# nianticlabs/simplerecon

Hardware: AMD Instinct MI355X
Metric: depth frames/sec (640x480, 7 src views, 64 planes) (higher is better)
Workload: dtype f32

## Files before the change

simplerecon_amd/csrc/sr_common.h:

```cpp
#pragma once
#include <hip/hip_runtime.h>
#include <stdint.h>

#include "simplerecon_hip.h"

#define SR_GEOM_STRIDE 20

#define SR_WAVE 64

int sr_opt(int id);

int sr_device_cus();

static inline int sr_hip_rc(hipError_t e) { return e == hipSuccess ? SR_OK : SR_ERR_HIP_BASE + (int)e; }

static inline size_t sr_align_up(size_t v, size_t a) { return (v + a - 1) / a * a; }

struct SrPlanes {
  const float* ptr;
  int64_t sb, sd, sy, sx;
};

struct SrVolumeOut {
  float* cv;
  int64_t sb, sd, sp;
  float* lowest;
  uint8_t* mask;
};

struct SrSample {
  float zp;
  float pix_x, pix_y;
  float w_nw, w_ne, w_sw, w_se;
  int o_nw, o_ne, o_sw, o_se;
};

typedef float sr_f2v __attribute__((ext_vector_type(2)));

__device__ __forceinline__ void sr_bilinear_taps(float ix, float iy, int h, int w, float& fx0, float& fy0, float& w_nw,
                                                 float& w_ne, float& w_sw, float& w_se) {
#pragma clang fp contract(off)
  const sr_f2v ixy = {ix, iy};
  fx0 = floorf(ix);
  fy0 = floorf(iy);
  const sr_f2v f0 = {fx0, fy0};
  const sr_f2v f1 = f0 + 1.0f;
  const float fx1 = f1.x, fy1 = f1.y;
  const float wm = (float)(w - 1), hm = (float)(h - 1);
  const bool vx0 = (fx0 >= 0.0f) & (fx0 <= wm), vx1 = (fx1 >= 0.0f) & (fx1 <= wm);
  const bool vy0 = (fy0 >= 0.0f) & (fy0 <= hm), vy1 = (fy1 >= 0.0f) & (fy1 <= hm);
  const sr_f2v a1 = f1 - ixy, a0 = ixy - f0;
  const sr_f2v wtop = sr_f2v{a1.x, a0.x} * a1.y;
  const sr_f2v wbot = sr_f2v{a1.x, a0.x} * a0.y;
  w_nw = (vx0 & vy0) ? wtop.x : 0.0f;
  w_ne = (vx1 & vy0) ? wtop.y : 0.0f;
  w_sw = (vx0 & vy1) ? wbot.x : 0.0f;
  w_se = (vx1 & vy1) ? wbot.y : 0.0f;
}

struct SrSampleXY {
  float zp, pix_x, pix_y;
  float ix, iy;
  float fx0, fy0;
  float w_nw, w_ne, w_sw, w_se;
};

__device__ __forceinline__ void sr_project_sample_xy(const float* __restrict__ g ,
                                                     float X0, float X1, float X2, int h, int w,
                                                     float inv_w, float inv_h, SrSampleXY& s) {
#pragma clang fp contract(off)
  const float eps = 1e-8f;
  const sr_f2v q01 = sr_f2v{g[0], g[4]} * X0 + sr_f2v{g[1], g[5]} * X1 + sr_f2v{g[2], g[6]} * X2 + sr_f2v{g[3], g[7]};
  const float q2 = g[8] * X0 + g[9] * X1 + g[10] * X2 + g[11];
  s.zp = q2 + eps;
  const float sc = (fabsf(q2) > eps) ? 1.0f / s.zp : 1.0f;
  const sr_f2v pix = q01 * sc;
  s.pix_x = pix.x;
  s.pix_y = pix.y;
  const sr_f2v uv = 2.0f * pix * sr_f2v{inv_w, inv_h} - 1.0f;
  const sr_f2v size = {(float)w, (float)h};
  const sr_f2v ixy = ((uv + 1.0f) * size - 1.0f) / 2.0f;
  s.ix = ixy.x;
  s.iy = ixy.y;
  sr_bilinear_taps(s.ix, s.iy, h, w, s.fx0, s.fy0, s.w_nw, s.w_ne, s.w_sw, s.w_se);
}

__device__ __forceinline__ void sr_project_sample(const float* __restrict__ g ,
                                                  float X0, float X1, float X2, int h, int w,
                                                  float inv_w, float inv_h, SrSample& s) {
  SrSampleXY c;
  sr_project_sample_xy(g, X0, X1, X2, h, w, inv_w, inv_h, c);
  s.zp = c.zp; s.pix_x = c.pix_x; s.pix_y = c.pix_y;
  s.w_nw = c.w_nw; s.w_ne = c.w_ne; s.w_sw = c.w_sw; s.w_se = c.w_se;
  const float wm = (float)(w - 1), hm = (float)(h - 1);
  const float fx1 = c.fx0 + 1.0f, fy1 = c.fy0 + 1.0f;
  const int x0 = (int)fminf(fmaxf(c.fx0, 0.0f), wm), x1 = (int)fminf(fmaxf(fx1, 0.0f), wm);
  const int y0 = (int)fminf(fmaxf(c.fy0, 0.0f), hm), y1 = (int)fminf(fmaxf(fy1, 0.0f), hm);
  s.o_nw = y0 * w + x0;
  s.o_ne = y0 * w + x1;
  s.o_sw = y1 * w + x0;
  s.o_se = y1 * w + x1;
}

__device__ __forceinline__ bool sr_in_bounds(const SrSample& s, int h, int w) {
  return (s.pix_x > 2.0f) & (s.pix_x < (float)(w - 2)) & (s.pix_y > 2.0f) & (s.pix_y < (float)(h - 2));
}

#ifdef __HIPCC__
__device__ __forceinline__ float sr_vmax(float a, float b) {
  float r;
  asm("v_max_f32 %0, %1, %2" : "=v"(r) : "v"(a), "v"(b));
  return r;
}
__device__ __forceinline__ float sr_vmin(float a, float b) {
  float r;
  asm("v_min_f32 %0, %1, %2" : "=v"(r) : "v"(a), "v"(b));
  return r;
}
__device__ __forceinline__ float sr_vmax_mfma(float a, float b) {
  float r;
  asm("v_max_f32 %0, %1, %2\n\ts_nop 1" : "=v"(r) : "v"(a), "v"(b));
  return r;
}
__device__ __forceinline__ float sr_activate(float v, float slope) {
  if (slope >= 0.0f) return fmaxf(v, 0.0f) + slope * fminf(v, 0.0f);
  if (slope < -1.5f) return v / (1.0f + __expf(-v));
  return v;
}
__device__ __forceinline__ float sr_uniform(float x) {
  return __builtin_bit_cast(float, __builtin_amdgcn_readfirstlane(__builtin_bit_cast(int, x)));
}
template <int N>
__device__ __forceinline__ void sr_activate_group(float (&v)[N], float slope) {
  if (slope >= 0.0f) {
    if (slope <= 1.0f) {
#pragma unroll
      for (int i = 0; i < N; ++i) v[i] = sr_vmax(v[i], slope * v[i]);
    } else {
#pragma unroll
      for (int i = 0; i < N; ++i) v[i] = sr_vmax(v[i], 0.0f) + slope * sr_vmin(v[i], 0.0f);
    }
  } else if (slope < -1.5f) {
#pragma unroll
    for (int i = 0; i < N; ++i) v[i] = v[i] / (1.0f + __expf(-v[i]));
  }
}
#endif

struct SrDotParams {
  const float* cur;
  const float* src_nhwc;
  const float* invK;
  const float* geom;
  SrPlanes planes;
  SrVolumeOut out;
  int B, K, h, w, D;
  float inv_w, inv_h;
};

static inline float* sr_ws_geom(void* workspace) { return (float*)sr_align_up((size_t)workspace, 256); }
static inline float* sr_ws_src_nhwc(void* workspace, int B, int K) {
  return (float*)((char*)sr_ws_geom(workspace) + sr_align_up((size_t)B * K * SR_GEOM_STRIDE * sizeof(float), 256));
}

static inline size_t sr_ws_nhwc_bytes(int B, int K, int C, int h, int w) {
  return sr_align_up((size_t)B * K * h * w * C * sizeof(float), 256);
}
static inline unsigned long long* sr_ws_keys(void* workspace, int B, int K, int C, int h, int w) {
  return (unsigned long long*)((char*)sr_ws_src_nhwc(workspace, B, K) + sr_ws_nhwc_bytes(B, K, C, h, w));
}

int sr_launch_dot_volume_lds(const SrDotParams& p, unsigned long long* keys, hipStream_t stream);
int sr_launch_geom(const float* K_src, const float* T_src_cur, const float* T_cur_src, float* geom,
                   int n, hipStream_t stream);
int sr_launch_argmax_planes(const float* cv, int64_t sb, int64_t sd, int64_t sp, SrPlanes planes, int B, int h, int w,
                            int D, float* lowest, hipStream_t stream);
int sr_launch_splitk_reduce(const float* part, int ksplit, int64_t part_stride, const float* bias, const float* res,
                            int64_t res_sb, int res_sp, float* out, int64_t out_sb, int out_sp, int B, int HW, int Cout,
                            float slope, hipStream_t stream);
int sr_launch_unpack_nhwc(const float* src_nhwc, float* dst_nchw, int images, int C, int npix, hipStream_t stream);
int sr_launch_pack_nhwc(const float* src_nchw, float* dst_nhwc, int images, int C, int npix,
                        hipStream_t stream);
```

simplerecon_amd/csrc/sr_mlp_volume.hip:

```cpp
#include <stdlib.h>
#include <string.h>

#include "sr_common.h"

typedef float f32x16 __attribute__((ext_vector_type(16)));

#define SR_HID 128
#define SR_VIEW_SLOTS 24
#define SR_INV_FIXED 20
#define SR_PLANE_CHUNK 8

static inline int sr_mlp_steps_var(int K) { return (SR_VIEW_SLOTS / 2) * K; }
static inline int sr_mlp_steps_inv(int K) { return (SR_INV_FIXED + 3 * K + 1) / 2; }
static inline int sr_mlp_steps1(int K) { return sr_mlp_steps_var(K) + sr_mlp_steps_inv(K); }
#define SR_MLP_STEPS2 65

static inline size_t sr_mlp_packed_floats(int K) { return (size_t)(sr_mlp_steps1(K) + SR_MLP_STEPS2) * 256 + 128 + 4; }

__global__ void sr_mlp_pack_kernel(const float* __restrict__ W1, const float* __restrict__ b1,
                                   const float* __restrict__ W2, const float* __restrict__ b2,
                                   const float* __restrict__ W3, const float* __restrict__ b3,
                                   float* __restrict__ packed, int K, int C) {
  const int steps_var = (SR_VIEW_SLOTS / 2) * K;
  const int steps1 = steps_var + (SR_INV_FIXED + 3 * K + 1) / 2;
  const int Cin = C * (K + 1) + 10 * K + 4;
  const int o_cur = K * C, o_mask = o_cur + C, o_z = o_mask + K, o_d = o_z + K, o_dot = o_d + 1;
  const int o_ang = o_dot + K, o_cray = o_ang + K, o_sray = o_cray + 3, o_pd = o_sray + 3 * K;
  const int o_rm = o_pd + K, o_tm = o_rm + K;
  const int total = (steps1 + SR_MLP_STEPS2) * 256 + 128 + 1;
  for (int e = blockIdx.x * blockDim.x + threadIdx.x; e < total; e += gridDim.x * blockDim.x) {
    float v = 0.0f;
    if (e < steps1 * 256) {
      const int t = e >> 8, lane = (e >> 2) & 63, mt = e & 3;
      const int row = 32 * mt + (lane & 31);
      int col = -1;
      if (t < steps_var) {
        const int slot = 2 * t + (lane >> 5);
        const int k = slot / SR_VIEW_SLOTS, s = slot - k * SR_VIEW_SLOTS;
        if (s < 16) col = k * C + s;
        else if (s == 16) col = o_mask + k;
        else if (s == 17) col = o_z + k;
        else if (s == 18) col = o_dot + k;
        else if (s == 19) col = o_ang + k;
        else if (s < 23) col = o_sray + 3 * k + (s - 20);
        else col = (k == 0) ? o_d : -1;
      } else {
        const int u = 2 * (t - steps_var) + (lane >> 5);
        if (u < 16) col = o_cur + u;
        else if (u < 19) col = o_cray + (u - 16);
        else if (u == 19) col = -2;
        else if (u < SR_INV_FIXED + 3 * K) {
          const int k = (u - SR_INV_FIXED) / 3, i = (u - SR_INV_FIXED) - 3 * k;
          col = (i == 0 ? o_pd : (i == 1 ? o_rm : o_tm)) + k;
        }
      }
      v = (col >= 0) ? W1[(size_t)row * Cin + col] : (col == -2 ? b1[row] : 0.0f);
    } else if (e < (steps1 + SR_MLP_STEPS2) * 256) {
      const int e2 = e - steps1 * 256;
      const int t = e2 >> 8, lane = (e2 >> 2) & 63, mt = e2 & 3;
      const int row = 32 * mt + (lane & 31);
      if (t < 64) {
        const int m = t >> 4, r = t & 15;
        const int f = 32 * m + (r & 3) + 8 * (r >> 2) + 4 * (lane >> 5);
        v = W2[(size_t)row * SR_HID + f];
      } else {
        v = (lane < 32) ? b2[row] : 0.0f;
      }
    } else if (e < (steps1 + SR_MLP_STEPS2) * 256 + 128) {
      const int i = e - (steps1 + SR_MLP_STEPS2) * 256;
      const int half = i >> 6, mt = (i >> 4) & 3, r = i & 15;
      v = W3[32 * mt + (r & 3) + 8 * (r >> 2) + 4 * half];
    } else {
      v = b3[0];
    }
    packed[e] = v;
  }
}


struct SrMlpParams {
  const float* cur;
  const float* src_nhwc;
  const float* invK;
  const float* geom;
  const float* packed;
  SrPlanes planes;
  SrVolumeOut out;
  int B, K, h, w, D;
  int tiles;
  int chunk, chunks;
  int vec_store;
  float inv_w, inv_h, slope;
};

__device__ __forceinline__ void sr_swap_halves(float fa, float fb, float& bP, float& bQ) {
  auto r = __builtin_amdgcn_permlane32_swap(__float_as_uint(fa), __float_as_uint(fb), false, false);
  bP = __uint_as_float(r[0]);
  bQ = __uint_as_float(r[1]);
}

#define SR_MFMA(a, b, c) __builtin_amdgcn_mfma_f32_32x32x2f32((a), (b), (c), 0, 0, 0)

__device__ __forceinline__ void sr_l1_step(f32x16 (&acc)[2][4], const float4 wA, float fa, float fb) {
  float bP, bQ;
  sr_swap_halves(fa, fb, bP, bQ);
  acc[0][0] = SR_MFMA(wA.x, bP, acc[0][0]);
  acc[1][0] = SR_MFMA(wA.x, bQ, acc[1][0]);
  acc[0][1] = SR_MFMA(wA.y, bP, acc[0][1]);
  acc[1][1] = SR_MFMA(wA.y, bQ, acc[1][1]);
  acc[0][2] = SR_MFMA(wA.z, bP, acc[0][2]);
  acc[1][2] = SR_MFMA(wA.z, bQ, acc[1][2]);
  acc[0][3] = SR_MFMA(wA.w, bP, acc[0][3]);
  acc[1][3] = SR_MFMA(wA.w, bQ, acc[1][3]);
}

__device__ __forceinline__ void sr_l1_step_init(f32x16 (&acc)[2][4], const f32x16 (&hc)[2][4], const float4 wA,
                                                float fa, float fb) {
  float bP, bQ;
  sr_swap_halves(fa, fb, bP, bQ);
  acc[0][0] = SR_MFMA(wA.x, bP, hc[0][0]);
  acc[1][0] = SR_MFMA(wA.x, bQ, hc[1][0]);
  acc[0][1] = SR_MFMA(wA.y, bP, hc[0][1]);
  acc[1][1] = SR_MFMA(wA.y, bQ, hc[1][1]);
  acc[0][2] = SR_MFMA(wA.z, bP, hc[0][2]);
  acc[1][2] = SR_MFMA(wA.z, bQ, hc[1][2]);
  acc[0][3] = SR_MFMA(wA.w, bP, hc[0][3]);
  acc[1][3] = SR_MFMA(wA.w, bQ, hc[1][3]);
}

#define SR_LDS_W3_FLOATS 256

template <bool W1_LDS, bool W2_LDS>
__global__ __launch_bounds__(256, 1) void sr_mlp_volume_kernel(SrMlpParams p) {
  extern __shared__ __attribute__((aligned(16))) float lds[];
  constexpr int C = 16;
  constexpr int VS = SR_VIEW_SLOTS / 2;
  const int lane = threadIdx.x & 63;
  const int steps_var = VS * p.K;
  const int steps1 = steps_var + (SR_INV_FIXED + 3 * p.K + 1) / 2;
  const float4* gW1 = reinterpret_cast<const float4*>(p.packed);
  const float4* gW1inv = gW1 + (size_t)steps_var * 64;
  const float4* gW2 = gW1 + (size_t)steps1 * 64;
  const float* gW3 = p.packed + (size_t)(steps1 + SR_MLP_STEPS2) * 256;

  for (int i = threadIdx.x; i < 129; i += blockDim.x) lds[i] = gW3[i];
  constexpr int W2_FLOATS = W2_LDS ? SR_MLP_STEPS2 * 256 : 0;
  if (W2_LDS) {
    float4* l4 = reinterpret_cast<float4*>(lds + SR_LDS_W3_FLOATS);
    for (int i = threadIdx.x; i < SR_MLP_STEPS2 * 64; i += blockDim.x) l4[i] = gW2[i];
  }
  if (W1_LDS) {
    float4* l4 = reinterpret_cast<float4*>(lds + SR_LDS_W3_FLOATS + W2_FLOATS);
    for (int i = threadIdx.x; i < steps_var * 64; i += blockDim.x) l4[i] = gW1[i];
  }
  __syncthreads();
  const float4* W1p = W1_LDS ? reinterpret_cast<const float4*>(lds + SR_LDS_W3_FLOATS + W2_FLOATS) : gW1;

  const int N = p.h * p.w;
  const long nunits = (long)p.B * p.tiles * p.chunks;
  long wave0 = (long)blockIdx.x * (blockDim.x >> 6) + (threadIdx.x >> 6);
  long nwaves = (long)gridDim.x * (blockDim.x >> 6);
  long unit_end = nunits;
  if ((gridDim.x & 7) == 0) {
    const long u8 = (nunits + 7) / 8;
    const int xcd = blockIdx.x & 7;
    nwaves = (long)(gridDim.x >> 3) * (blockDim.x >> 6);
    wave0 = xcd * u8 + (long)(blockIdx.x >> 3) * (blockDim.x >> 6) + (threadIdx.x >> 6);
    unit_end = min(nunits, (xcd + 1) * u8);
  }
  const int half = lane >> 5;

  for (long unit = wave0; unit < unit_end; unit += nwaves) {
    const int chunk = (int)(unit % p.chunks);
    const long tb = unit / p.chunks;
    const int tile = (int)(tb % p.tiles);
    const int b = (int)(tb / p.tiles);
    const int j0 = chunk * p.chunk, j1 = min(p.D, j0 + p.chunk);
    const int pix = tile * 64 + lane;
    const bool active = pix < N;
    const int pc = active ? pix : N - 1;
    const int y = pc / p.w, x = pc - y * p.w;
    const float* plane_ptr = p.planes.ptr + b * p.planes.sb + y * p.planes.sy + x * p.planes.sx;
    const float* geom_b = p.geom + (size_t)b * p.K * SR_GEOM_STRIDE;
    const float* src_b = p.src_nhwc + (size_t)b * p.K * N * C;

    float cur[C];
#pragma unroll
    for (int c = 0; c < C; ++c) cur[c] = p.cur[((size_t)b * C + c) * N + pc];

    float r0, r1, r2;
    {
#pragma clang fp contract(off)
      const float* iK = p.invK + 16 * (size_t)b;
      const float px = (float)x + 0.5f, py = (float)y + 0.5f;
      r0 = iK[0] * px + iK[1] * py + iK[2];
      r1 = iK[4] * px + iK[5] * py + iK[6];
      r2 = iK[8] * px + iK[9] * py + iK[10];
    }
    float cr0, cr1, cr2, crn0, crn1, crn2;
    {
#pragma clang fp contract(off)
      const float d0 = plane_ptr[0];
      const float X0 = d0 * r0, X1 = d0 * r1, X2 = d0 * r2;
      const float cden = fmaxf(sqrtf((X0 * X0 + X1 * X1) + X2 * X2), 1e-12f);
      cr0 = X0 / cden; cr1 = X1 / cden; cr2 = X2 / cden;
      const float n1 = fmaxf(sqrtf((cr0 * cr0 + cr1 * cr1) + cr2 * cr2), 1e-5f);
      crn0 = cr0 / n1; crn1 = cr1 / n1; crn2 = cr2 / n1;
    }

    f32x16 hc[2][4];
#pragma unroll
    for (int g = 0; g < 2; ++g)
#pragma unroll
      for (int m = 0; m < 4; ++m)
#pragma unroll
        for (int r = 0; r < 16; ++r) hc[g][m][r] = 0.0f;
    {
      const float4* wi = gW1inv + lane;
#pragma unroll
      for (int t = 0; t < 8; ++t) sr_l1_step(hc, wi[t * 64], cur[2 * t], cur[2 * t + 1]);
      sr_l1_step(hc, wi[8 * 64], cr0, cr1);
      sr_l1_step(hc, wi[9 * 64], cr2, 1.0f);
      const int npose = 3 * p.K;
#pragma unroll 1
      for (int u = 0; u < npose; u += 2) {
        const int ka = u / 3, ia = u - 3 * ka, kb = (u + 1) / 3, ib = (u + 1) - 3 * kb;
        const float fa = geom_b[ka * SR_GEOM_STRIDE + 15 + ia];
        const float fb = (u + 1 < npose) ? geom_b[kb * SR_GEOM_STRIDE + 15 + ib] : 0.0f;
        sr_l1_step(hc, wi[(size_t)(10 + (u >> 1)) * 64], fa, fb);
      }
    }

    SrSample smp;
    float4 taps[16];
    float f[SR_VIEW_SLOTS], fn[SR_VIEW_SLOTS];
    float X0, X1, X2, d;
    bool any_depth, any_bounds;
    auto issue_view = [&](int k) {
      sr_project_sample(geom_b + k * SR_GEOM_STRIDE, X0, X1, X2, p.h, p.w, p.inv_w, p.inv_h, smp);
      const float* img = src_b + (size_t)k * N * C;
      const float4* t_nw = reinterpret_cast<const float4*>(img + (size_t)smp.o_nw * C);
      const float4* t_ne = reinterpret_cast<const float4*>(img + (size_t)smp.o_ne * C);
      const float4* t_sw = reinterpret_cast<const float4*>(img + (size_t)smp.o_sw * C);
      const float4* t_se = reinterpret_cast<const float4*>(img + (size_t)smp.o_se * C);
#pragma unroll
      for (int i = 0; i < 4; ++i) {
        taps[i] = t_nw[i]; taps[4 + i] = t_ne[i]; taps[8 + i] = t_sw[i]; taps[12 + i] = t_se[i];
      }
    };
    float rv0, rv1, rv2, rsd, rdot;
#define SR_RAY_A(o, g, kview)                                                                 \
    {                                                                                         \
      _Pragma("clang fp contract(off)")                                                       \
      rv0 = X0 - (g)[12]; rv1 = X1 - (g)[13]; rv2 = X2 - (g)[14];                              \
      rsd = fmaxf(sqrtf((rv0 * rv0 + rv1 * rv1) + rv2 * rv2), 1e-12f);                         \
      (o)[23] = ((kview) == 0) ? d : 0.0f;       \
    }
#define SR_RAY_B(o)                                                                           \
    {                                                                                         \
      _Pragma("clang fp contract(off)")                                                       \
      const float rinv = 1.0f / rsd;                                                          \
      (o)[20] = rv0 * rinv; (o)[21] = rv1 * rinv; (o)[22] = rv2 * rinv;                        \
    }
#define SR_RAY_C(o)                                                                           \
    {                                                                                         \
      _Pragma("clang fp contract(off)")                                                       \
      const float n2 = fmaxf(sqrtf(((o)[20] * (o)[20] + (o)[21] * (o)[21]) + (o)[22] * (o)[22]), 1e-5f); \
      (o)[19] = ((crn0 * (o)[20] + crn1 * (o)[21]) + crn2 * (o)[22]) * (1.0f / n2);            \
    }
#define SR_INTERP2(o, i, lo)         \
    {                                                                                         \
      const float4 a = taps[i], bq = taps[4 + (i)], c4 = taps[8 + (i)], d4 = taps[12 + (i)];   \
      const sr_f2v ta = (lo) == 0 ? sr_f2v{a.x, a.y} : sr_f2v{a.z, a.w};                       \
      const sr_f2v tb = (lo) == 0 ? sr_f2v{bq.x, bq.y} : sr_f2v{bq.z, bq.w};                   \
      const sr_f2v tc = (lo) == 0 ? sr_f2v{c4.x, c4.y} : sr_f2v{c4.z, c4.w};                   \
      const sr_f2v td = (lo) == 0 ? sr_f2v{d4.x, d4.y} : sr_f2v{d4.z, d4.w};                   \
      const sr_f2v r2 = __builtin_elementwise_fma(sr_f2v{smp.w_se, smp.w_se}, td,              \
                        __builtin_elementwise_fma(sr_f2v{smp.w_sw, smp.w_sw}, tc,              \
                        __builtin_elementwise_fma(sr_f2v{smp.w_ne, smp.w_ne}, tb,              \
                                                  sr_f2v{smp.w_nw, smp.w_nw} * ta)));          \
      (o)[4 * (i) + 2 * (lo) + 0] = r2.x;                                                     \
      (o)[4 * (i) + 2 * (lo) + 1] = r2.y;                                                     \
    }
#define SR_DOT(o)                                                                             \
    {                                                                                         \
      rdot = 0.0f;                                                                            \
      _Pragma("unroll") for (int c = 0; c < 16; ++c) rdot = fmaf((o)[c], cur[c], rdot);        \
      const bool front = smp.zp > 0.0f;                                                       \
      any_depth |= front;                                                                     \
      any_bounds |= sr_in_bounds(smp, p.h, p.w);                                              \
      (o)[16] = front ? 1.0f : 0.0f;                       \
      (o)[17] = smp.zp;                                    \
      (o)[18] = front ? rdot : 0.0f;                 \
    }
#define SR_SB __builtin_amdgcn_sched_barrier(0);

    constexpr bool CST_LDS = !W1_LDS;
    const int cst_base = SR_LDS_W3_FLOATS + W2_FLOATS +
                         __builtin_amdgcn_readfirstlane(threadIdx.x >> 6) * (SR_PLANE_CHUNK * 64);
    float cst[SR_PLANE_CHUNK];
#pragma unroll
    for (int q = 0; q < SR_PLANE_CHUNK; ++q) cst[q] = 0.0f;
#pragma unroll 1
    for (int j = j0; j < j1; ++j) {
      d = plane_ptr[j * p.planes.sd];
      {
#pragma clang fp contract(off)
        X0 = d * r0; X1 = d * r1; X2 = d * r2;
      }
      any_depth = false; any_bounds = false;
      f32x16 acc[2][4];

      {
        issue_view(0);
        SR_RAY_A(f, geom_b, 0) SR_RAY_B(f) SR_RAY_C(f)
        SR_INTERP2(f, 0, 0) SR_INTERP2(f, 0, 1) SR_INTERP2(f, 1, 0) SR_INTERP2(f, 1, 1)
        SR_INTERP2(f, 2, 0) SR_INTERP2(f, 2, 1) SR_INTERP2(f, 3, 0) SR_INTERP2(f, 3, 1)
        SR_DOT(f)
      }
#define SR_STEP(t)                                           \
        wN = wk[((t) + 1 < VS ? (t) + 1 : (t)) * 64];       \
        sr_l1_step(acc, wA, f[2 * (t)], f[2 * (t) + 1]);     \
        wA = wN;
#define SR_VIEW_BODY(FIRST)                                                            \
        {                                                                              \
          const int kn = min(k + 1, p.K - 1);  \
          const float* g = geom_b + kn * SR_GEOM_STRIDE;                               \
          issue_view(kn);                                                              \
          const float4* wk = W1p + (size_t)(VS * k) * 64 + lane;                       \
          float4 wA = wk[0], wN;                                                       \
          SR_SB                                                                        \
          if (FIRST) { wN = wk[64]; sr_l1_step_init(acc, hc, wA, f[0], f[1]); wA = wN; } \
          else { SR_STEP(0) }                                                          \
          SR_RAY_A(fn, g, kn) SR_SB                                                    \
          SR_STEP(1) SR_RAY_B(fn) SR_SB                                                \
          SR_STEP(2) SR_RAY_C(fn) SR_SB                                                \
          SR_STEP(3) SR_SB  \
          SR_STEP(4) SR_SB                                                             \
          SR_STEP(5) SR_SB                                                             \
          SR_STEP(6) SR_SB                                                             \
          SR_STEP(7) SR_INTERP2(fn, 0, 0) SR_INTERP2(fn, 0, 1) SR_SB                   \
          SR_STEP(8) SR_INTERP2(fn, 1, 0) SR_INTERP2(fn, 1, 1) SR_SB                   \
          SR_STEP(9) SR_INTERP2(fn, 2, 0) SR_INTERP2(fn, 2, 1) SR_SB                   \
          SR_STEP(10) SR_INTERP2(fn, 3, 0) SR_SB                                       \
          SR_STEP(11) SR_INTERP2(fn, 3, 1) SR_DOT(fn) SR_SB                            \
          _Pragma("unroll") for (int t = 0; t < SR_VIEW_SLOTS; ++t) f[t] = fn[t];      \
        }
      {
        const int k = 0;
        SR_VIEW_BODY(true)
      }
#pragma unroll 1
      for (int k = 1; k < p.K; ++k) SR_VIEW_BODY(false)

      f32x16 acc2[2][4];
      const f32x16 zero16 = {0.f, 0.f, 0.f, 0.f, 0.f, 0.f, 0.f, 0.f, 0.f, 0.f, 0.f, 0.f, 0.f, 0.f, 0.f, 0.f};
      const float4* w2 = (W2_LDS ? reinterpret_cast<const float4*>(lds + SR_LDS_W3_FLOATS) : gW2) + lane;
      if (!W2_LDS) asm volatile("" : "+v"(w2));
      float4 wn0 = w2[0], wn1 = w2[64], wn2 = w2[128];
#pragma unroll
      for (int t = 0; t < 64; ++t) {
        const float4 wA = wn0;
        wn0 = wn1;
        wn1 = wn2;
        wn2 = w2[(size_t)min(t + 3, 64) * 64];
        const float aP = acc[0][t >> 4][t & 15], aQ = acc[1][t >> 4][t & 15];
        const float bP = sr_vmax_mfma(aP, p.slope * aP), bQ = sr_vmax_mfma(aQ, p.slope * aQ);
        acc2[0][0] = SR_MFMA(wA.x, bP, t == 0 ? zero16 : acc2[0][0]);
        acc2[1][0] = SR_MFMA(wA.x, bQ, t == 0 ? zero16 : acc2[1][0]);
        acc2[0][1] = SR_MFMA(wA.y, bP, t == 0 ? zero16 : acc2[0][1]);
        acc2[1][1] = SR_MFMA(wA.y, bQ, t == 0 ? zero16 : acc2[1][1]);
        acc2[0][2] = SR_MFMA(wA.z, bP, t == 0 ? zero16 : acc2[0][2]);
        acc2[1][2] = SR_MFMA(wA.z, bQ, t == 0 ? zero16 : acc2[1][2]);
        acc2[0][3] = SR_MFMA(wA.w, bP, t == 0 ? zero16 : acc2[0][3]);
        acc2[1][3] = SR_MFMA(wA.w, bQ, t == 0 ? zero16 : acc2[1][3]);
      }
      {
        const float4 wA = wn0;
        const float one = half ? 0.0f : 1.0f;
        acc2[0][0] = SR_MFMA(wA.x, one, acc2[0][0]);
        acc2[1][0] = SR_MFMA(wA.x, one, acc2[1][0]);
        acc2[0][1] = SR_MFMA(wA.y, one, acc2[0][1]);
        acc2[1][1] = SR_MFMA(wA.y, one, acc2[1][1]);
        acc2[0][2] = SR_MFMA(wA.z, one, acc2[0][2]);
        acc2[1][2] = SR_MFMA(wA.z, one, acc2[1][2]);
        acc2[0][3] = SR_MFMA(wA.w, one, acc2[0][3]);
        acc2[1][3] = SR_MFMA(wA.w, one, acc2[1][3]);
      }

      const float4* w3 = reinterpret_cast<const float4*>(lds + half * 64);
      sr_f2v oPQ = {0.0f, 0.0f};
      const sr_f2v slope2 = {p.slope, p.slope};
#pragma unroll
      for (int m = 0; m < 4; ++m)
#pragma unroll
        for (int q = 0; q < 4; ++q) {
          const float4 wv = w3[m * 4 + q];
          const float wr[4] = {wv.x, wv.y, wv.z, wv.w};
#pragma unroll
          for (int i = 0; i < 4; ++i) {
            const sr_f2v h2 = {acc2[0][m][4 * q + i], acc2[1][m][4 * q + i]};
            const sr_f2v s2 = slope2 * h2;
            oPQ = __builtin_elementwise_fma(sr_f2v{wr[i], wr[i]}, sr_f2v{sr_vmax(h2.x, s2.x), sr_vmax(h2.y, s2.y)}, oPQ);
          }
        }
      float oP = oPQ.x, oQ = oPQ.y;
      oP += __shfl_xor(oP, 32);
      oQ += __shfl_xor(oQ, 32);
      const float cost = (half ? oQ : oP) + lds[128];

      if (p.vec_store) {
        if (CST_LDS) lds[cst_base + (j - j0) * 64 + lane] = cost;
        else {
#pragma unroll
          for (int q = 0; q < SR_PLANE_CHUNK; ++q) cst[q] = (j - j0 == q) ? cost : cst[q];
        }
      }
      if (active) {
        if (!p.vec_store) p.out.cv[b * p.out.sb + j * p.out.sd + (int64_t)pix * p.out.sp] = cost;
        if (j == p.D - 1 && p.out.mask) p.out.mask[(size_t)b * N + pix] = (uint8_t)(any_depth && any_bounds);
      }
    }
    if (p.vec_store && active) {
      float* row = p.out.cv + b * p.out.sb + (int64_t)pix * p.out.sp + j0;
      if (CST_LDS) {
#pragma unroll
        for (int q = 0; q < SR_PLANE_CHUNK; ++q) cst[q] = lds[cst_base + q * 64 + lane];
      }
#pragma unroll
      for (int q = 0; q < SR_PLANE_CHUNK; q += 4) {
        if (j0 + q + 4 <= j1) *reinterpret_cast<float4*>(row + q) = make_float4(cst[q], cst[q + 1], cst[q + 2], cst[q + 3]);
        else {
#pragma unroll
          for (int i = 0; i < 4; ++i)
            if (j0 + q + i < j1) row[q + i] = cst[q + i];
        }
      }
    }
  }
}

typedef unsigned sr_u4v __attribute__((ext_vector_type(4)));

template <int FMT> struct SrSplitFmt;
template <> struct SrSplitFmt<1> {
  typedef __bf16 e2 __attribute__((ext_vector_type(2)));
  typedef __bf16 e8 __attribute__((ext_vector_type(8)));
  static __device__ __forceinline__ void split(float a, float b, unsigned& hi, unsigned& lo) {
    const sr_f2v v = {a, b};
    hi = __builtin_bit_cast(unsigned, __builtin_convertvector(v, e2));
    const sr_f2v v0 = {__uint_as_float(hi << 16), __uint_as_float(hi & 0xffff0000u)};
    lo = __builtin_bit_cast(unsigned, __builtin_convertvector(v - v0, e2));
  }
  static __device__ __forceinline__ f32x16 mfma(sr_u4v a, sr_u4v b, f32x16 c) {
    return __builtin_amdgcn_mfma_f32_32x32x16_bf16(__builtin_bit_cast(e8, a), __builtin_bit_cast(e8, b), c, 0, 0, 0);
  }
};
template <> struct SrSplitFmt<2> {
  typedef _Float16 e2 __attribute__((ext_vector_type(2)));
  typedef _Float16 e8 __attribute__((ext_vector_type(8)));
  static __device__ __forceinline__ void split(float a, float b, unsigned& hi, unsigned& lo) {
    const sr_f2v v = {a, b};
    const e2 h = __builtin_convertvector(v, e2);
    hi = __builtin_bit_cast(unsigned, h);
    lo = __builtin_bit_cast(unsigned, __builtin_convertvector(v - __builtin_convertvector(h, sr_f2v), e2));
  }
  static __device__ __forceinline__ f32x16 mfma(sr_u4v a, sr_u4v b, f32x16 c) {
    return __builtin_amdgcn_mfma_f32_32x32x16_f16(__builtin_bit_cast(e8, a), __builtin_bit_cast(e8, b), c, 0, 0, 0);
  }
};

#define SR_SPL_TAB 512
#define SR_SPL_W2_WORDS 16384
#define SR_SPL_VIEW_WORDS 3072

template <int FMT>
__global__ void sr_mlp_pack_split_kernel(const float* __restrict__ W1, const float* __restrict__ b1,
                                         const float* __restrict__ W2, const float* __restrict__ b2,
                                         const float* __restrict__ W3, const float* __restrict__ b3,
                                         float* __restrict__ packed, int K, int C) {
  typedef SrSplitFmt<FMT> S;
  const int steps_var = (SR_VIEW_SLOTS / 2) * K;
  const int steps_inv = (SR_INV_FIXED + 3 * K + 1) / 2;
  const int steps1 = steps_var + steps_inv;
  const int Cin = C * (K + 1) + 10 * K + 4;
  const int o_cur = K * C, o_mask = o_cur + C, o_z = o_mask + K, o_d = o_z + K, o_dot = o_d + 1;
  const int o_ang = o_dot + K, o_cray = o_ang + K, o_sray = o_cray + 3, o_pd = o_sray + 3 * K;
  const int o_rm = o_pd + K, o_tm = o_rm + K;
  unsigned* pk = reinterpret_cast<unsigned*>(packed);
  auto var_col = [&](int k, int s) {
    if (s < 16) return k * C + s;
    if (s == 16) return o_mask + k;
    if (s == 17) return o_z + k;
    if (s == 18) return o_dot + k;
    if (s == 19) return o_ang + k;
    if (s < 23) return o_sray + 3 * k + (s - 20);
    return (k == 0) ? o_d : -1;
  };
  auto put = [&](size_t word, int piece, float wa, float wb) {
    unsigned hi, lo;
    S::split(wa, wb, hi, lo);
    pk[word] = piece ? lo : hi;
  };
  const int total = (steps1 + SR_MLP_STEPS2) * 256 + 128 + 1;
  for (int e = blockIdx.x * blockDim.x + threadIdx.x; e < total; e += gridDim.x * blockDim.x) {
    if (e < steps_var * 256) {
      const int k = e / SR_SPL_VIEW_WORDS, q = e - k * SR_SPL_VIEW_WORDS;
      int mt, piece, lane, dw, slot0;
      if (q < 2048) { mt = q >> 9; piece = (q >> 8) & 1; lane = (q >> 2) & 63; dw = q & 3; slot0 = 8 * (lane >> 5) + 2 * dw; }
      else { const int q2 = q - 2048; mt = q2 >> 8; piece = (q2 >> 7) & 1; lane = (q2 >> 2) & 31; dw = q2 & 3; slot0 = 16 + 2 * dw; }
      const int row = 32 * mt + (lane & 31);
      const int ca = var_col(k, slot0), cb = var_col(k, slot0 + 1);
      put(e, piece, ca >= 0 ? W1[(size_t)row * Cin + ca] : 0.0f, cb >= 0 ? W1[(size_t)row * Cin + cb] : 0.0f);
    } else if (e < steps1 * 256) {
      const int e1 = e - steps_var * 256;
      const int t = e1 >> 8, lane = (e1 >> 2) & 63, mt = e1 & 3;
      const int row = 32 * mt + (lane & 31);
      const int u = 2 * t + (lane >> 5);
      int col = -1;
      if (u < 16) col = o_cur + u;
      else if (u < 19) col = o_cray + (u - 16);
      else if (u == 19) col = -2;
      else if (u < SR_INV_FIXED + 3 * K) {
        const int k = (u - SR_INV_FIXED) / 3, i = (u - SR_INV_FIXED) - 3 * k;
        col = (i == 0 ? o_pd : (i == 1 ? o_rm : o_tm)) + k;
      }
      packed[e] = (col >= 0) ? W1[(size_t)row * Cin + col] : (col == -2 ? b1[row] : 0.0f);
    } else if (e < steps1 * 256 + SR_SPL_W2_WORDS) {
      const int q = e - steps1 * 256;
      const int s = q >> 11, mt = (q >> 9) & 3, piece = (q >> 8) & 1, lane = (q >> 2) & 63, dw = q & 3;
      const int row = 32 * mt + (lane & 31);
      auto feat = [&](int i) { const int r = 8 * (s & 1) + i; return 32 * (s >> 1) + (r & 3) + 8 * (r >> 2) + 4 * (lane >> 5); };
      put(e, piece, W2[(size_t)row * SR_HID + feat(2 * dw)], W2[(size_t)row * SR_HID + feat(2 * dw + 1)]);
    } else if (e < (steps1 + SR_MLP_STEPS2) * 256) {
      const int i = e - steps1 * 256 - SR_SPL_W2_WORDS;
      const int half = i >> 6, mt = (i >> 4) & 3, r = i & 15;
      packed[e] = (i < 128) ? b2[32 * mt + (r & 3) + 8 * (r >> 2) + 4 * half] : 0.0f;
    } else if (e < (steps1 + SR_MLP_STEPS2) * 256 + 128) {
      const int i = e - (steps1 + SR_MLP_STEPS2) * 256;
      const int half = i >> 6, mt = (i >> 4) & 3, r = i & 15;
      packed[e] = W3[32 * mt + (r & 3) + 8 * (r >> 2) + 4 * half];
    } else {
      packed[e] = b3[0];
    }
  }
}

__device__ __forceinline__ void sr_swap_halves_u4(const sr_u4v fa, const sr_u4v fb, sr_u4v& bP, sr_u4v& bQ) {
#pragma unroll
  for (int i = 0; i < 4; ++i) {
    auto r = __builtin_amdgcn_permlane32_swap(fa[i], fb[i], false, false);
    bP[i] = r[0];
    bQ[i] = r[1];
  }
}

template <int FMT, int INIT>
__device__ __forceinline__ void sr_spl_step(f32x16 (&acc)[2][4], const f32x16 (&c0)[2][4], const sr_u4v* aw, int ls,
                                            const sr_u4v bPh, const sr_u4v bPl, const sr_u4v bQh, const sr_u4v bQl) {
  typedef SrSplitFmt<FMT> S;
  sr_u4v ah[4], al[4];
#pragma unroll
  for (int m = 0; m < 4; ++m) { ah[m] = aw[(2 * m) * ls]; al[m] = aw[(2 * m + 1) * ls]; }
#pragma unroll
  for (int m = 0; m < 4; ++m) {
    const f32x16 zero16 = {0.f, 0.f, 0.f, 0.f, 0.f, 0.f, 0.f, 0.f, 0.f, 0.f, 0.f, 0.f, 0.f, 0.f, 0.f, 0.f};
    acc[0][m] = S::mfma(ah[m], bPh, INIT == 1 ? c0[0][m] : (INIT == 2 ? zero16 : acc[0][m]));
    acc[1][m] = S::mfma(ah[m], bQh, INIT == 1 ? c0[1][m] : (INIT == 2 ? zero16 : acc[1][m]));
  }
#pragma unroll
  for (int m = 0; m < 4; ++m) {
    acc[0][m] = S::mfma(ah[m], bPl, acc[0][m]);
    acc[1][m] = S::mfma(ah[m], bQl, acc[1][m]);
  }
#pragma unroll
  for (int m = 0; m < 4; ++m) {
    acc[0][m] = S::mfma(al[m], bPh, acc[0][m]);
    acc[1][m] = S::mfma(al[m], bQh, acc[1][m]);
  }
}

template <int FMT>
__global__ __launch_bounds__(256, 1) void sr_mlp_volume_split_kernel(SrMlpParams p) {
  typedef SrSplitFmt<FMT> S;
  extern __shared__ __attribute__((aligned(16))) float lds[];
  constexpr int C = 16;
  const int lane = threadIdx.x & 63;
  const int steps_var = (SR_VIEW_SLOTS / 2) * p.K;
  const int steps1 = steps_var + (SR_INV_FIXED + 3 * p.K + 1) / 2;
  const float4* gW1inv = reinterpret_cast<const float4*>(p.packed) + (size_t)steps_var * 64;
  const float* gW2 = p.packed + (size_t)steps1 * 256;
  const float* gW3 = p.packed + (size_t)(steps1 + SR_MLP_STEPS2) * 256;

  for (int i = threadIdx.x; i < 129; i += blockDim.x) lds[i] = gW3[i];
  for (int i = threadIdx.x; i < 128; i += blockDim.x) lds[256 + i] = gW2[SR_SPL_W2_WORDS + i];
  {
    float4* l4 = reinterpret_cast<float4*>(lds + SR_SPL_TAB);
    const float4* g4 = reinterpret_cast<const float4*>(gW2);
    for (int i = threadIdx.x; i < SR_SPL_W2_WORDS / 4; i += blockDim.x) l4[i] = g4[i];
    l4 += SR_SPL_W2_WORDS / 4;
    g4 = reinterpret_cast<const float4*>(p.packed);
    for (int i = threadIdx.x; i < p.K * (SR_SPL_VIEW_WORDS / 4); i += blockDim.x) l4[i] = g4[i];
  }
  __syncthreads();
  const sr_u4v* W2s = reinterpret_cast<const sr_u4v*>(lds + SR_SPL_TAB);
  const sr_u4v* W1s = W2s + SR_SPL_W2_WORDS / 4;

  const int N = p.h * p.w;
  const long nunits = (long)p.B * p.tiles * p.chunks;
  long wave0 = (long)blockIdx.x * (blockDim.x >> 6) + (threadIdx.x >> 6);
  long nwaves = (long)gridDim.x * (blockDim.x >> 6);
  long unit_end = nunits;
  if ((gridDim.x & 7) == 0) {
    const long u8 = (nunits + 7) / 8;
    const int xcd = blockIdx.x & 7;
    nwaves = (long)(gridDim.x >> 3) * (blockDim.x >> 6);
    wave0 = xcd * u8 + (long)(blockIdx.x >> 3) * (blockDim.x >> 6) + (threadIdx.x >> 6);
    unit_end = min(nunits, (xcd + 1) * u8);
  }
  const int half = lane >> 5;
  const sr_u4v zero4 = {0u, 0u, 0u, 0u};

  for (long unit = wave0; unit < unit_end; unit += nwaves) {
    const int chunk = (int)(unit % p.chunks);
    const long tb = unit / p.chunks;
    const int tile = (int)(tb % p.tiles);
    const int b = (int)(tb / p.tiles);
    const int j0 = chunk * p.chunk, j1 = min(p.D, j0 + p.chunk);
    const int pix = tile * 64 + lane;
    const bool active = pix < N;
    const int pc = active ? pix : N - 1;
    const int y = pc / p.w, x = pc - y * p.w;
    const float* plane_ptr = p.planes.ptr + b * p.planes.sb + y * p.planes.sy + x * p.planes.sx;
    const float* geom_b = p.geom + (size_t)b * p.K * SR_GEOM_STRIDE;
    const float* src_b = p.src_nhwc + (size_t)b * p.K * N * C;

    float cur[C];
#pragma unroll
    for (int c = 0; c < C; ++c) cur[c] = p.cur[((size_t)b * C + c) * N + pc];

    float r0, r1, r2;
    {
#pragma clang fp contract(off)
      const float* iK = p.invK + 16 * (size_t)b;
      const float px = (float)x + 0.5f, py = (float)y + 0.5f;
      r0 = iK[0] * px + iK[1] * py + iK[2];
      r1 = iK[4] * px + iK[5] * py + iK[6];
      r2 = iK[8] * px + iK[9] * py + iK[10];
    }
    float cr0, cr1, cr2, crn0, crn1, crn2;
    {
#pragma clang fp contract(off)
      const float d0 = plane_ptr[0];
      const float X0 = d0 * r0, X1 = d0 * r1, X2 = d0 * r2;
      const float cden = fmaxf(sqrtf((X0 * X0 + X1 * X1) + X2 * X2), 1e-12f);
      cr0 = X0 / cden; cr1 = X1 / cden; cr2 = X2 / cden;
// ... 333 lines not shown
```

Before: 313.8.

## Skip tap loads and interpolation MFMAs for wave-wide out-of-bounds views

Computes a per-sample any_tap flag and uses a wave ballot to detect source views where no lane has any valid bilinear tap. For such views it skips the feature gathers, the interpolation, and the first eight MLP layer-1 steps whose inputs would be zero, using four specialised body variants chosen per (current, next) liveness. It also rotates the plane-chunk assignment across tiles, which probably spreads load across waves. Code size and branching increase, and the gain depends on how often whole waves fall outside a source view.

```diff
diff --git a/simplerecon_amd/csrc/sr_common.h b/simplerecon_amd/csrc/sr_common.h
--- a/simplerecon_amd/csrc/sr_common.h
+++ b/simplerecon_amd/csrc/sr_common.h
@@ -33,12 +33,13 @@
   float pix_x, pix_y;
   float w_nw, w_ne, w_sw, w_se;
   int o_nw, o_ne, o_sw, o_se;
+  bool any_tap;
 };
 
 typedef float sr_f2v __attribute__((ext_vector_type(2)));
 
 __device__ __forceinline__ void sr_bilinear_taps(float ix, float iy, int h, int w, float& fx0, float& fy0, float& w_nw,
-                                                 float& w_ne, float& w_sw, float& w_se) {
+                                                 float& w_ne, float& w_sw, float& w_se, bool& any_tap) {
 #pragma clang fp contract(off)
   const sr_f2v ixy = {ix, iy};
   fx0 = floorf(ix);
@@ -56,6 +57,12 @@
   w_ne = (vx1 & vy0) ? wtop.y : 0.0f;
   w_sw = (vx0 & vy1) ? wbot.x : 0.0f;
   w_se = (vx1 & vy1) ? wbot.y : 0.0f;
+  any_tap = (vx0 | vx1) & (vy0 | vy1);
+}
+__device__ __forceinline__ void sr_bilinear_taps(float ix, float iy, int h, int w, float& fx0, float& fy0, float& w_nw,
+                                                 float& w_ne, float& w_sw, float& w_se) {
+  bool any_tap;
+  sr_bilinear_taps(ix, iy, h, w, fx0, fy0, w_nw, w_ne, w_sw, w_se, any_tap);
 }
 
 struct SrSampleXY {
@@ -63,6 +70,7 @@
   float ix, iy;
   float fx0, fy0;
   float w_nw, w_ne, w_sw, w_se;
+  bool any_tap;
 };
 
 __device__ __forceinline__ void sr_project_sample_xy(const float* __restrict__ g ,
@@ -82,7 +90,7 @@
   const sr_f2v ixy = ((uv + 1.0f) * size - 1.0f) / 2.0f;
   s.ix = ixy.x;
   s.iy = ixy.y;
-  sr_bilinear_taps(s.ix, s.iy, h, w, s.fx0, s.fy0, s.w_nw, s.w_ne, s.w_sw, s.w_se);
+  sr_bilinear_taps(s.ix, s.iy, h, w, s.fx0, s.fy0, s.w_nw, s.w_ne, s.w_sw, s.w_se, s.any_tap);
 }
 
 __device__ __forceinline__ void sr_project_sample(const float* __restrict__ g ,
@@ -92,6 +100,7 @@
   sr_project_sample_xy(g, X0, X1, X2, h, w, inv_w, inv_h, c);
   s.zp = c.zp; s.pix_x = c.pix_x; s.pix_y = c.pix_y;
   s.w_nw = c.w_nw; s.w_ne = c.w_ne; s.w_sw = c.w_sw; s.w_se = c.w_se;
+  s.any_tap = c.any_tap;
   const float wm = (float)(w - 1), hm = (float)(h - 1);
   const float fx1 = c.fx0 + 1.0f, fy1 = c.fy0 + 1.0f;
   const int x0 = (int)fminf(fmaxf(c.fx0, 0.0f), wm), x1 = (int)fminf(fmaxf(fx1, 0.0f), wm);
diff --git a/simplerecon_amd/csrc/sr_mlp_volume.hip b/simplerecon_amd/csrc/sr_mlp_volume.hip
--- a/simplerecon_amd/csrc/sr_mlp_volume.hip
+++ b/simplerecon_amd/csrc/sr_mlp_volume.hip
@@ -128,6 +128,12 @@
   acc[1][3] = SR_MFMA(wA.w, bQ, hc[1][3]);
 }
 
+__device__ __forceinline__ int sr_opaque(bool flag) {
+  int v = __builtin_amdgcn_readfirstlane((int)flag);
+  asm volatile("" : "+s"(v));
+  return v;
+}
+
 #define SR_LDS_W3_FLOATS 256
 
 template <bool W1_LDS, bool W2_LDS>
@@ -158,21 +164,24 @@
 
   const int N = p.h * p.w;
   const long nunits = (long)p.B * p.tiles * p.chunks;
-  long wave0 = (long)blockIdx.x * (blockDim.x >> 6) + (threadIdx.x >> 6);
-  long nwaves = (long)gridDim.x * (blockDim.x >> 6);
+  constexpr int WPB = 4;
+  const int wid = __builtin_amdgcn_readfirstlane(threadIdx.x >> 6);
+  long wave0 = (long)blockIdx.x * WPB + wid;
+  long nwaves = (long)gridDim.x * WPB;
   long unit_end = nunits;
   if ((gridDim.x & 7) == 0) {
     const long u8 = (nunits + 7) / 8;
     const int xcd = blockIdx.x & 7;
-    nwaves = (long)(gridDim.x >> 3) * (blockDim.x >> 6);
-    wave0 = xcd * u8 + (long)(blockIdx.x >> 3) * (blockDim.x >> 6) + (threadIdx.x >> 6);
+    nwaves = (long)(gridDim.x >> 3) * WPB;
+    wave0 = xcd * u8 + (long)(blockIdx.x >> 3) * WPB + wid;
     unit_end = min(nunits, (xcd + 1) * u8);
   }
   const int half = lane >> 5;
 
+  const int rot = (int)max(1L, nwaves / p.chunks);
   for (long unit = wave0; unit < unit_end; unit += nwaves) {
-    const int chunk = (int)(unit % p.chunks);
     const long tb = unit / p.chunks;
+    const int chunk = (int)((unit % p.chunks + tb / rot) % p.chunks);
     const int tile = (int)(tb % p.tiles);
     const int b = (int)(tb / p.tiles);
     const int j0 = chunk * p.chunk, j1 = min(p.D, j0 + p.chunk);
@@ -233,11 +242,16 @@
 
     SrSample smp;
     float4 taps[16];
-    float f[SR_VIEW_SLOTS], fn[SR_VIEW_SLOTS];
     float X0, X1, X2, d;
     bool any_depth, any_bounds;
-    auto issue_view = [&](int k) {
-      sr_project_sample(geom_b + k * SR_GEOM_STRIDE, X0, X1, X2, p.h, p.w, p.inv_w, p.inv_h, smp);
+    float gt0, gt1, gt2;
+    auto project_view = [&](int k) -> bool {
+      const float* g = geom_b + k * SR_GEOM_STRIDE;
+      gt0 = g[12]; gt1 = g[13]; gt2 = g[14];
+      sr_project_sample(g, X0, X1, X2, p.h, p.w, p.inv_w, p.inv_h, smp);
+      return __builtin_amdgcn_ballot_w64(active & smp.any_tap) == 0;
+    };
+    auto load_taps = [&](int k) {
       const float* img = src_b + (size_t)k * N * C;
       const float4* t_nw = reinterpret_cast<const float4*>(img + (size_t)smp.o_nw * C);
       const float4* t_ne = reinterpret_cast<const float4*>(img + (size_t)smp.o_ne * C);
@@ -249,13 +263,15 @@
       }
     };
     float rv0, rv1, rv2, rsd, rdot;
-#define SR_RAY_A(o, g, kview)                                                                 \
+#define SR_RAY_A_T(o, t0, t1, t2, kview)                                                      \
     {                                                                                         \
       _Pragma("clang fp contract(off)")                                                       \
-      rv0 = X0 - (g)[12]; rv1 = X1 - (g)[13]; rv2 = X2 - (g)[14];                              \
+      rv0 = X0 - (t0); rv1 = X1 - (t1); rv2 = X2 - (t2);                                       \
       rsd = fmaxf(sqrtf((rv0 * rv0 + rv1 * rv1) + rv2 * rv2), 1e-12f);                         \
       (o)[23] = ((kview) == 0) ? d : 0.0f;       \
     }
+#define SR_RAY_A(o, g, kview) SR_RAY_A_T(o, (g)[12], (g)[13], (g)[14], kview)
+#define SR_RAY_A0(o, kview) SR_RAY_A_T(o, gt0, gt1, gt2, kview)
 #define SR_RAY_B(o)                                                                           \
     {                                                                                         \
       _Pragma("clang fp contract(off)")                                                       \
@@ -293,11 +309,20 @@
       (o)[17] = smp.zp;                                    \
       (o)[18] = front ? rdot : 0.0f;                 \
     }
+#define SR_DOT_DEAD(o)   \
+    {                                                                                         \
+      const bool front = smp.zp > 0.0f;                                                       \
+      any_depth |= front;                                                                     \
+      any_bounds |= sr_in_bounds(smp, p.h, p.w);                                              \
+      (o)[16] = front ? 1.0f : 0.0f;                                                          \
+      (o)[17] = smp.zp;                                                                       \
+      (o)[18] = 0.0f;                                                                         \
+    }
 #define SR_SB __builtin_amdgcn_sched_barrier(0);
 
     constexpr bool CST_LDS = !W1_LDS;
     const int cst_base = SR_LDS_W3_FLOATS + W2_FLOATS +
-                         __builtin_amdgcn_readfirstlane(threadIdx.x >> 6) * (SR_PLANE_CHUNK * 64);
+                         wid * (SR_PLANE_CHUNK * 64);
     float cst[SR_PLANE_CHUNK];
 #pragma unroll
     for (int q = 0; q < SR_PLANE_CHUNK; ++q) cst[q] = 0.0f;
@@ -310,48 +335,76 @@
       }
       any_depth = false; any_bounds = false;
       f32x16 acc[2][4];
-
-      {
-        issue_view(0);
-        SR_RAY_A(f, geom_b, 0) SR_RAY_B(f) SR_RAY_C(f)
+      float f[SR_VIEW_SLOTS], fn[SR_VIEW_SLOTS];
+
+      bool dc = project_view(0), dn;
+      if (!dc) {
+        load_taps(0);
+        SR_RAY_A0(f, 0) SR_RAY_B(f) SR_RAY_C(f)
         SR_INTERP2(f, 0, 0) SR_INTERP2(f, 0, 1) SR_INTERP2(f, 1, 0) SR_INTERP2(f, 1, 1)
         SR_INTERP2(f, 2, 0) SR_INTERP2(f, 2, 1) SR_INTERP2(f, 3, 0) SR_INTERP2(f, 3, 1)
         SR_DOT(f)
+      } else {
+        SR_RAY_A0(f, 0) SR_RAY_B(f) SR_RAY_C(f)
+        SR_DOT_DEAD(f)
+        f[0] = f[1] = 0.0f;
       }
 #define SR_STEP(t)                                           \
         wN = wk[((t) + 1 < VS ? (t) + 1 : (t)) * 64];       \
         sr_l1_step(acc, wA, f[2 * (t)], f[2 * (t) + 1]);     \
         wA = wN;
-#define SR_VIEW_BODY(FIRST)                                                            \
+#define SR_IF_LIVE(ND, x) if (!(ND)) { x }
+#define SR_VIEW_BODY(FIRST, CD, ND)                                                    \
         {                                                                              \
-          const int kn = min(k + 1, p.K - 1);  \
-          const float* g = geom_b + kn * SR_GEOM_STRIDE;                               \
-          issue_view(kn);                                                              \
+          if (!(ND)) load_taps(kn);                                                    \
           const float4* wk = W1p + (size_t)(VS * k) * 64 + lane;                       \
-          float4 wA = wk[0], wN;                                                       \
+          float4 wA = wk[((CD) ? 8 : 0) * 64 + ((FIRST) ? 64 : 0)], wN;                \
           SR_SB                                                                        \
-          if (FIRST) { wN = wk[64]; sr_l1_step_init(acc, hc, wA, f[0], f[1]); wA = wN; } \
-          else { SR_STEP(0) }                                                          \
-          SR_RAY_A(fn, g, kn) SR_SB                                                    \
-          SR_STEP(1) SR_RAY_B(fn) SR_SB                                                \
-          SR_STEP(2) SR_RAY_C(fn) SR_SB                                                \
-          SR_STEP(3) SR_SB  \
-          SR_STEP(4) SR_SB                                                             \
-          SR_STEP(5) SR_SB                                                             \
-          SR_STEP(6) SR_SB                                                             \
-          SR_STEP(7) SR_INTERP2(fn, 0, 0) SR_INTERP2(fn, 0, 1) SR_SB                   \
-          SR_STEP(8) SR_INTERP2(fn, 1, 0) SR_INTERP2(fn, 1, 1) SR_SB                   \
-          SR_STEP(9) SR_INTERP2(fn, 2, 0) SR_INTERP2(fn, 2, 1) SR_SB                   \
-          SR_STEP(10) SR_INTERP2(fn, 3, 0) SR_SB                                       \
-          SR_STEP(11) SR_INTERP2(fn, 3, 1) SR_DOT(fn) SR_SB                            \
-          _Pragma("unroll") for (int t = 0; t < SR_VIEW_SLOTS; ++t) f[t] = fn[t];      \
+          if (!(CD)) {                                                                 \
+            if (!(FIRST)) { SR_STEP(0) SR_RAY_A0(fn, kn) SR_SB }                     \
+            SR_STEP(1) if (FIRST) { SR_RAY_A0(fn, kn) } SR_RAY_B(fn) SR_SB           \
+            SR_STEP(2) SR_RAY_C(fn) SR_SB                                              \
+            SR_STEP(3) SR_SB                                                           \
+            SR_STEP(4) SR_SB                                                           \
+            SR_STEP(5) SR_SB                                                           \
+            SR_STEP(6) SR_SB                                                           \
+            SR_STEP(7) SR_IF_LIVE(ND, SR_INTERP2(fn, 0, 0) SR_INTERP2(fn, 0, 1)) SR_SB \
+            SR_STEP(8) SR_IF_LIVE(ND, SR_INTERP2(fn, 1, 0) SR_INTERP2(fn, 1, 1)) SR_SB \
+            SR_STEP(9) SR_IF_LIVE(ND, SR_INTERP2(fn, 2, 0) SR_INTERP2(fn, 2, 1)) SR_SB \
+            SR_STEP(10) SR_IF_LIVE(ND, SR_INTERP2(fn, 3, 0)) SR_SB                     \
+            SR_STEP(11) if (ND) { SR_DOT_DEAD(fn) } else { SR_INTERP2(fn, 3, 1) SR_DOT(fn) } SR_SB \
+          } else {                                                                     \
+            if (!(FIRST)) { SR_STEP(8) SR_RAY_A0(fn, kn) SR_SB }                     \
+            SR_STEP(9) if (FIRST) { SR_RAY_A0(fn, kn) } SR_RAY_B(fn) SR_RAY_C(fn) SR_SB \
+            SR_STEP(10) SR_IF_LIVE(ND, SR_INTERP2(fn, 0, 0) SR_INTERP2(fn, 0, 1)       \
+                                       SR_INTERP2(fn, 1, 0) SR_INTERP2(fn, 1, 1)) SR_SB \
+            SR_STEP(11) if (ND) { SR_DOT_DEAD(fn) } else {                             \
+              SR_INTERP2(fn, 2, 0) SR_INTERP2(fn, 2, 1) SR_INTERP2(fn, 3, 0) SR_INTERP2(fn, 3, 1) SR_DOT(fn) } SR_SB \
+          }                                                                            \
+          _Pragma("unroll") for (int t = (ND) ? 16 : 0; t < SR_VIEW_SLOTS; ++t) f[t] = fn[t]; \
+        }
+#define SR_VIEW(FIRST)                                                                 \
+        {                                                                              \
+          const int kn = min(k + 1, p.K - 1);                                          \
+          dn = project_view(kn) | (k + 1 >= p.K);                                      \
+          const int ll = sr_opaque(!dc & !dn), ld = sr_opaque(!dc & dn);               \
+          const int dl = sr_opaque(dc & !dn), dd = sr_opaque(dc & dn);                 \
+          if (ll) SR_VIEW_BODY(FIRST, false, false)                                    \
+          if (ld) SR_VIEW_BODY(FIRST, false, true)                                     \
+          if (dl) SR_VIEW_BODY(FIRST, true, false)                                     \
+          if (dd) SR_VIEW_BODY(FIRST, true, true)                                      \
+          dc = dn;                                                                     \
         }
       {
+        const float4 w0 = W1p[(size_t)(dc ? 8 * 64 : 0) + lane];
+        sr_l1_step_init(acc, hc, w0, dc ? f[16] : f[0], dc ? f[17] : f[1]);
+      }
+      {
         const int k = 0;
-        SR_VIEW_BODY(true)
+        SR_VIEW(true)
       }
 #pragma unroll 1
-      for (int k = 1; k < p.K; ++k) SR_VIEW_BODY(false)
+      for (int k = 1; k < p.K; ++k) SR_VIEW(false)
 
       f32x16 acc2[2][4];
       const f32x16 zero16 = {0.f, 0.f, 0.f, 0.f, 0.f, 0.f, 0.f, 0.f, 0.f, 0.f, 0.f, 0.f, 0.f, 0.f, 0.f, 0.f};
```

After: 322.3 (median of 6 runs). +2.7%, better.
